# KORandi/bullet-js

Measured on AMD Instinct MI355X. Metric: CRDT field-merges/s, higher is better.
Workload: dtype int64

## Files before the change

bullet-js_amd/csrc/merge_kernels.h:

```cpp
#pragma once
#include "slot.h"
#include "../../include/bmx.h"

namespace bmx {

__device__ unsigned long long g_wait_ticks = 6000000000ull;
__device__ __forceinline__ bool wait_gave_up(unsigned long long t0, const uint32_t* status) {
  return wall_clock64() - t0 > g_wait_ticks || (__hip_atomic_load(status, __ATOMIC_RELAXED, __HIP_MEMORY_SCOPE_AGENT) & ST_SPIN) != 0;
}
constexpr int PART_MAX_SHARDS = 16;
struct SeqPtrs { unsigned long long* p[PART_MAX_SHARDS]; };

struct MergeArgs {
  Slot* slots;
  uint64_t nslots;
  const uint64_t* id;
  const uint32_t* field;
  const int64_t* ts;
  const int64_t* val;
  const bmx_delta_rec* recs;
  uint32_t n;
  uint32_t epoch;
  uint32_t* next;
  uint32_t* blk_follow;
  uint8_t* wflag;
  uint8_t* flags;
  uint32_t* slot_of;
  uint32_t* blk_info;
  unsigned long long* shard_ctr;
  uint32_t* status;
  uint32_t* blk_next;
  uint32_t blk_ents;
  uint32_t force;
  unsigned long long* started = nullptr;
  unsigned long long started_val = 0;
  const unsigned long long* k3_done = nullptr;
  unsigned long long k3_wait = 0;
  uint32_t* fld_out = nullptr;
  uint32_t log_slots = 0;
  SeqPtrs notify{}; uint32_t n_notify = 0; unsigned long long notify_value = 0;
  const unsigned long long* tail_words = nullptr; uint32_t tail_n = 0; unsigned long long tail_at_least = 0; unsigned long long* tail_diag = nullptr;
};

constexpr uint8_t W_NONE = 0, W_WINNER = 1, W_PENDING = 2, W_FIRST = 4;
constexpr uint8_t W_CREATED = 8;
constexpr uint8_t W_FIRSTWRITE = 16;
constexpr uint32_t BLK_COUNT = 0x7FFFFFFFu;
constexpr uint32_t CTR_SHARDS = 256, CTR_STRIDE = 16;

template <bool AOS>
__device__ __forceinline__ void load_delta(const MergeArgs& A, uint32_t j, uint64_t& id, uint32_t& field, int64_t& ts, int64_t& val) {
  if (AOS) {
    const uint4* p = reinterpret_cast<const uint4*>(A.recs + j);
    uint4 lo = p[0], hi = p[1];
    id = u64_of(lo.x, lo.y);
    field = lo.z;
    ts = i64_of(hi.x, hi.y);
    val = i64_of(hi.z, hi.w);
  } else {
    id = A.id[j]; field = A.field[j]; ts = A.ts[j]; val = A.val[j];
  }
}
template <bool AOS>
__device__ __forceinline__ void load_delta_tv(const MergeArgs& A, uint32_t j, int64_t& ts, int64_t& val) {
  if (AOS) {
    uint4 hi = reinterpret_cast<const uint4*>(A.recs + j)[1];
    ts = i64_of(hi.x, hi.y);
    val = i64_of(hi.z, hi.w);
  } else {
    ts = A.ts[j]; val = A.val[j];
  }
}

__device__ __forceinline__ void store_tv(Slot* sl, int64_t ts, int64_t val) {
  reinterpret_cast<uint4*>(sl)[1] = uint4_of((uint64_t)ts, (uint64_t)val);
}

template <bool UNIQUE>
__device__ __forceinline__ bool probe_or_insert(const MergeArgs& A, uint32_t tag, uint64_t id, uint32_t field, uint64_t& slot_out,
                                                bool& is_new, bool& created, uint32_t& prev_head, int64_t& cts, int64_t& cval) {
  created = false;
  ProbeSeq<4> ps(id, field, A.nslots);
  uint64_t p = 0;
  for (uint32_t round = 0; round < 256; ++round) {
    Slot* wait_on = nullptr;
    uint64_t s = 0;
    int done = 0;
    for (; p < A.nslots; ++p) {
      s = ps.slot();
      Slot* sl = A.slots + s;
      const uint4* q = reinterpret_cast<const uint4*>(sl);
      uint4 lo = q[0], hi = q[1];
      uint64_t sid = (uint64_t)lo.x | ((uint64_t)lo.y << 32);
      uint32_t sf = lo.z;
      bool fresh = false;
      if (sid == EMPTY_ID) {
        unsigned long long old = atomicCAS(reinterpret_cast<unsigned long long*>(&sl->id), (unsigned long long)EMPTY_ID, (unsigned long long)id);
        if (old == EMPTY_ID) {
          __hip_atomic_store(reinterpret_cast<unsigned long long*>(&sl->field), (unsigned long long)field | ((unsigned long long)(UNIQUE ? 0u : tag) << 32),
                             __ATOMIC_RELAXED, __HIP_MEMORY_SCOPE_AGENT);
          prev_head = 0;
          created = true;
          slot_out = s; is_new = true; cts = TS_NEW; cval = 0;
          done = 1;
          break;
        }
        sid = old;
        sf = FIELD_PENDING;
        fresh = true;
      }
      if (sid == id) {
        if (sf == FIELD_PENDING) { wait_on = sl; break; }
        if (sf == field) {
          int64_t t = (int64_t)((uint64_t)hi.x | ((uint64_t)hi.y << 32));
          slot_out = s;
          is_new = fresh || t == TS_NEW || ts_mark(t) == (tag >> IDX_BITS);
          cts = is_new ? TS_NEW : ts_value(t);
          cval = (int64_t)((uint64_t)hi.z | ((uint64_t)hi.w << 32));
          done = 1;
          break;
        }
      }
      ps.next();
    }
    if (done) return true;
    if (!wait_on) { atomicOr(A.status, ST_FULL); return false; }
    __builtin_amdgcn_wave_barrier();
    uint32_t sf = FIELD_PENDING, spins = 0;
    do {
      sf = __hip_atomic_load(&wait_on->field, __ATOMIC_RELAXED, __HIP_MEMORY_SCOPE_AGENT);
      if (sf != FIELD_PENDING) break;
      __builtin_amdgcn_s_sleep(1);
    } while (++spins < (1u << 22));
    if (sf == FIELD_PENDING) { atomicOr(A.status, ST_SPIN); return false; }
    if (sf == field) {
      slot_out = s; is_new = true; cts = TS_NEW; cval = 0;
      return true;
    }
    ps.next(); ++p;
  }
  atomicOr(A.status, ST_SPIN);
  return false;
}

template <int MODE, bool UNIQUE, bool TEAM = false>
__device__ __forceinline__ void decide_and_claim(const MergeArgs& A, const uint32_t j, const uint64_t s, const bool is_new, const bool created, uint32_t prev,
                                                 const int64_t cts, const int64_t cval, const int64_t a, const int64_t v,
                                                 uint32_t& fl, uint32_t& wf, bool& conflict) {
  const uint32_t tag = (A.epoch << IDX_BITS) | j;
  const int c = (is_new || A.force) ? 1 : lexcmp(a, v, cts, cval);
  if (c < 0) {
    fl = BMX_FLAG_CURRENT | (a < cts ? BMX_FLAG_HISTORICAL : 0u);
    return;
  }
  Slot* sl = A.slots + s;
  if (!TEAM && !created && !UNIQUE) prev = atomicExch(&sl->head, tag);
  if ((prev >> IDX_BITS) != A.epoch) {
    if (!UNIQUE) wf = W_FIRST;
    if (A.log_slots) A.slot_of[j] = (uint32_t)s;
    if (is_new) {
      const int64_t t0 = (MODE == BMX_INSERT_REFERENCE) ? 2 : a;
      store_tv(sl, t0 | ((int64_t)A.epoch << TS_MARK_SHIFT), v);
      wf |= W_WINNER | W_CREATED | W_FIRSTWRITE; fl = BMX_FLAG_INCOMING;
    } else if (c > 0) {
      if (!TEAM) store_tv(sl, a, v);
      wf |= W_WINNER; fl = BMX_FLAG_INCOMING;
    }
  } else {
    A.next[prev & IDX_MASK] = tag;
    A.slot_of[prev & IDX_MASK] = (uint32_t)s;
    A.blk_follow[(prev & IDX_MASK) >> 8] = A.epoch;
    wf = W_PENDING; conflict = true;
    fl = c > 0 ? BMX_FLAG_INCOMING : 0u;
  }
}

__device__ __forceinline__ uint32_t team_claim(const MergeArgs& A, const uint32_t j, const uint32_t s, const uint32_t field, const int64_t a, const int64_t v,
                                               const bool want, const bool wr) {
  const uint32_t lane = lane_id(), role = lane & 3u;
  const unsigned long long mw = __ballot(want), mv = __ballot(wr);
  uint32_t prev = 0;
#pragma unroll
  for (uint32_t p = 0; p < 4; p++) {
    if (!((mw >> (16u * p)) & 0xFFFFull)) continue;
    const uint32_t src = 16u * p + (lane >> 2);
    const uint32_t ss = (uint32_t)__shfl((int)s, (int)src), sf = (uint32_t)__shfl((int)field, (int)src);
    const uint64_t sa = u64_of((uint32_t)__shfl((int)lo32((uint64_t)a), (int)src), (uint32_t)__shfl((int)hi32((uint64_t)a), (int)src));
    const uint64_t sv = u64_of((uint32_t)__shfl((int)lo32((uint64_t)v), (int)src), (uint32_t)__shfl((int)hi32((uint64_t)v), (int)src));
    const bool on = role == 0 ? ((mw >> src) & 1ull) != 0 : (role != 3u && ((mv >> src) & 1ull) != 0);
    const uint64_t opnd = role == 0 ? u64_of(sf, (A.epoch << IDX_BITS) | (j - lane + src)) : (role == 1 ? sa : sv);
    unsigned long long old = 0;
    if (on) old = __hip_atomic_exchange(reinterpret_cast<unsigned long long*>(A.slots + ss) + 1 + role, (unsigned long long)opnd, __ATOMIC_RELAXED, __HIP_MEMORY_SCOPE_AGENT);
    const uint32_t got = (uint32_t)__shfl((int)hi32(old), (int)(4u * (lane & 15u)));
    if ((lane >> 4) == p) prev = got;
  }
  return prev;
}

template <bool AOS, int MODE, bool UNIQUE, int NT, bool TEAM = false>
__device__ __forceinline__ void probe_apply_body(const MergeArgs& A) {
  static_assert(!(TEAM && UNIQUE), "a unique-key batch claims nothing");
  const uint32_t j = blockIdx.x * (uint32_t)NT + threadIdx.x;
  if (A.started && j == 0) __hip_atomic_store(A.started, A.started_val, __ATOMIC_RELAXED, __HIP_MEMORY_SCOPE_AGENT);
  if (A.n_notify && j < A.n_notify && A.notify.p[j]) __hip_atomic_store(A.notify.p[j], A.notify_value, __ATOMIC_RELAXED, __HIP_MEMORY_SCOPE_SYSTEM);
  for (uint32_t t = j; t < A.blk_ents; t += gridDim.x * (uint32_t)NT) A.blk_next[t] = 0u;
  const bool active = j < A.n;
  uint64_t id = EMPTY_ID; uint32_t field = 0; int64_t a = 0, v = 0;
  if (active) load_delta<AOS>(A, j, id, field, a, v);
  if (A.fld_out && active) A.fld_out[j] = field;
  const bool pad = AOS && id == EMPTY_ID;
  const bool valid = active && id != EMPTY_ID && field != FIELD_PENDING && a >= 0 && a <= TS_MAX && ((v >= -VAL_MAX && v <= VAL_MAX) || (A.force && v == VAL_DELETED));
  if (active && !valid && !pad) atomicOr(A.status, ST_RANGE);
  uint32_t fl = 0, wf = W_NONE;
  bool conflict = false, created = false;
  if (TEAM) {
    bool is_new = false, located = false; int64_t cts = 0, cval = 0; uint64_t s = 0; uint32_t prev = 0;
    if (valid) located = probe_or_insert<UNIQUE>(A, (A.epoch << IDX_BITS) | j, id, field, s, is_new, created, prev, cts, cval);
    const int c = !located ? -1 : ((is_new || A.force) ? 1 : lexcmp(a, v, cts, cval));
    const bool want = c >= 0 && !created;
    const uint32_t got = team_claim(A, j, (uint32_t)s, field, a, v, want, want && c > 0 && !is_new);
    if (want) prev = got;
    if (located) decide_and_claim<MODE, UNIQUE, true>(A, j, s, is_new, created, prev, cts, cval, a, v, fl, wf, conflict);
  } else if (valid) {
    bool is_new; int64_t cts, cval; uint64_t s; uint32_t prev = 0;
    if (probe_or_insert<UNIQUE>(A, (A.epoch << IDX_BITS) | j, id, field, s, is_new, created, prev, cts, cval))
      decide_and_claim<MODE, UNIQUE>(A, j, s, is_new, created, prev, cts, cval, a, v, fl, wf, conflict);
  }
  if (active) {
    A.wflag[j] = (uint8_t)wf;
    if (A.flags) A.flags[j] = (uint8_t)fl;
  }
  const uint32_t nc = (uint32_t)__popcll(__ballot(created)), nx = (uint32_t)__popcll(__ballot(conflict));
  const uint32_t nw = (uint32_t)__popcll(__ballot((wf & W_WINNER) != 0));
  if (lane_id() == 0) {
    if (nw) atomicAdd(&A.blk_info[j >> 8], nw);
    if (nc | nx) {
      unsigned long long* ctr = A.shard_ctr + (size_t)((j >> 6) & (CTR_SHARDS - 1)) * CTR_STRIDE;
      if (nc) atomicAdd(ctr + 0, (unsigned long long)nc);
      if (nx) atomicAdd(ctr + 1, (unsigned long long)nx);
    }
  }
}

template <bool AOS, int MODE, bool UNIQUE, int NT, bool TEAM = false>
__global__ __launch_bounds__(NT) void k_probe_apply(MergeArgs A) { probe_apply_body<AOS, MODE, UNIQUE, NT, TEAM>(A); }
template <bool AOS, int MODE, bool UNIQUE, int NT, bool TEAM = false>
__global__ __launch_bounds__(NT) __attribute__((amdgpu_waves_per_eu(1, 6))) void k_probe_apply_w6(MergeArgs A) { probe_apply_body<AOS, MODE, UNIQUE, NT, TEAM>(A); }
template <bool AOS, int MODE, bool UNIQUE, int NT, bool TEAM = false>
__global__ __launch_bounds__(NT) __attribute__((amdgpu_waves_per_eu(1, 5))) void k_probe_apply_w5(MergeArgs A) { probe_apply_body<AOS, MODE, UNIQUE, NT, TEAM>(A); }
template <bool AOS, int MODE, bool UNIQUE, int NT, bool TEAM = false>
__global__ __launch_bounds__(NT) __attribute__((amdgpu_waves_per_eu(1, 4))) void k_probe_apply_w4(MergeArgs A) { probe_apply_body<AOS, MODE, UNIQUE, NT, TEAM>(A); }
template <bool AOS, int MODE, bool UNIQUE, int NT, bool TEAM = false>
__global__ __launch_bounds__(NT) __attribute__((amdgpu_waves_per_eu(1, 3))) void k_probe_apply_w3(MergeArgs A) { probe_apply_body<AOS, MODE, UNIQUE, NT, TEAM>(A); }


struct Top2 {
  int64_t t1 = INT64_MIN, v1 = INT64_MIN, t2 = INT64_MIN, v2 = INT64_MIN;
  uint32_t o1 = ~0u, o2 = ~0u;
  __device__ __forceinline__ void add(uint32_t idx, int64_t t, int64_t v) {
    int c1 = o1 == ~0u ? 1 : lexcmp(t, v, t1, v1);
    if (c1 > 0 || (c1 == 0 && idx < o1)) {
      if (o1 != ~0u) { int c2 = o2 == ~0u ? 1 : lexcmp(t1, v1, t2, v2); if (c2 > 0 || (c2 == 0 && o1 < o2)) { t2 = t1; v2 = v1; o2 = o1; } }
      t1 = t; v1 = v; o1 = idx;
    } else {
      int c2 = o2 == ~0u ? 1 : lexcmp(t, v, t2, v2);
      if (c2 > 0 || (c2 == 0 && idx < o2)) { t2 = t; v2 = v; o2 = idx; }
    }
  }
  __device__ __forceinline__ bool best_except(uint32_t skip, int64_t& t, int64_t& v, uint32_t& o) const {
    const bool use2 = o1 == skip;
    o = use2 ? o2 : o1;
    if (o == ~0u) return false;
    t = use2 ? t2 : t1; v = use2 ? v2 : v1;
    return true;
  }
};

template <bool AOS, int MODE>
__device__ __forceinline__ void resolve_one(const MergeArgs& A, const uint32_t j) {
  if (j >= A.n) return;
  const uint8_t wf = A.wflag[j];
  if (!(wf & W_FIRST)) return;
  uint32_t nx = A.next[j];
  if ((nx >> IDX_BITS) != A.epoch) return;
  int64_t t, v; load_delta_tv<AOS>(A, j, t, v);
  Slot* sl = A.slots + A.slot_of[j];
  const uint4 hi = reinterpret_cast<const uint4*>(sl)[1];
  const int64_t tsw = i64_of(hi.x, hi.y);
  const bool is_new = tsw == TS_NEW || ts_mark(tsw) == A.epoch;
  const uint32_t base_owner = (wf & W_WINNER) ? j : ~0u;
  int64_t bt, bv;
  uint32_t owner, created_by = ~0u;
  if (!is_new) {
    bt = t; bv = v; owner = base_owner;
    uint32_t idx = j, steps = 0;
    for (;;) {
      if (idx != j) {
        const bool gt = t > bt || (t == bt && v > bv);
        const bool eq = t == bt && v == bv;
        if (gt) { bt = t; bv = v; owner = idx; }
        else if (eq && owner != ~0u && idx < owner) owner = idx;
      }
      if ((nx >> IDX_BITS) != A.epoch) break;
      idx = nx & IDX_MASK;
      nx = A.next[idx]; load_delta_tv<AOS>(A, idx, t, v);
      if (++steps > A.n) { atomicOr(A.status, ST_SPIN); return; }
    }
  } else {
    uint32_t j0 = j;
    int64_t v_j0 = v, t_j0 = t;
    Top2 top;
    {
      uint32_t idx = j, steps = 0;
      for (;;) {
        if (idx <= j0) { j0 = idx; t_j0 = t; v_j0 = v; }
        top.add(idx, t, v);
        if ((nx >> IDX_BITS) != A.epoch) break;
        idx = nx & IDX_MASK;
        nx = A.next[idx]; load_delta_tv<AOS>(A, idx, t, v);
        if (++steps > A.n) { atomicOr(A.status, ST_SPIN); return; }
      }
    }
    bt = (MODE == BMX_INSERT_REFERENCE) ? 2 : t_j0; bv = v_j0; owner = j0; created_by = j0;
    int64_t tm, vm; uint32_t om;
    if (top.best_except(j0, tm, vm, om) && lexcmp(tm, vm, bt, bv) > 0) { bt = tm; bv = vm; owner = om; }
  }
  store_tv(sl, is_new ? (bt | ((int64_t)A.epoch << TS_MARK_SHIFT)) : bt, bv);
  if (base_owner != owner) {
    if (base_owner != ~0u) { A.wflag[base_owner] = W_NONE; atomicSub(&A.blk_info[base_owner >> 8], 1u); }
    if (owner != ~0u) {
      A.wflag[owner] = is_new ? (uint8_t)(W_WINNER | W_CREATED | (owner == created_by ? W_FIRSTWRITE : 0)) : W_WINNER; atomicAdd(&A.blk_info[owner >> 8], 1u);
      A.slot_of[owner] = A.slot_of[j];
    }
  } else if (is_new && owner != ~0u) {
    A.wflag[owner] = (uint8_t)(W_FIRST | W_WINNER | W_CREATED | (owner == created_by ? W_FIRSTWRITE : 0));
  }
  if (owner != ~0u && A.flags) A.flags[owner] = (uint8_t)BMX_FLAG_INCOMING;
}

template <bool AOS, int MODE>
__global__ __launch_bounds__(256) void k_resolve_lists(MergeArgs A) {
  if (A.blk_follow[blockIdx.x] == A.epoch) resolve_one<AOS, MODE>(A, blockIdx.x * 256u + threadIdx.x);
  if (A.k3_done && blockIdx.x == 0 && threadIdx.x == 0) {
    const unsigned long long t0 = wall_clock64();
    while (__hip_atomic_load(A.k3_done, __ATOMIC_RELAXED, __HIP_MEMORY_SCOPE_AGENT) < A.k3_wait) {
      __builtin_amdgcn_s_sleep(8);
      if (wait_gave_up(t0, A.status)) { atomicOr(A.status, ST_SPIN); break; }
    }
  }
  if (A.tail_n && blockIdx.x == 0 && threadIdx.x < A.tail_n) {
    const unsigned long long t0 = wall_clock64();
    unsigned long long seen;
    while ((seen = __hip_atomic_load(A.tail_words + threadIdx.x, __ATOMIC_RELAXED, __HIP_MEMORY_SCOPE_SYSTEM)) < A.tail_at_least) {
      __builtin_amdgcn_s_sleep(8);
      if (wait_gave_up(t0, A.status)) {
        if (A.tail_diag && !A.tail_diag[0]) { A.tail_diag[0] = (unsigned long long)(uintptr_t)(A.tail_words + threadIdx.x); A.tail_diag[1] = A.tail_at_least; A.tail_diag[2] = seen; }
        atomicOr(A.status, ST_SPIN);
        break;
      }
    }
  }
}

constexpr uint32_t STRICT_NO_ROW = 0xFFFFFFFFu;

template <bool AOS>
__global__ __launch_bounds__(256) void k_probe_link_strict(MergeArgs A) {
  const uint32_t j = blockIdx.x * 256u + threadIdx.x;
  const bool active = j < A.n;
  uint64_t id = EMPTY_ID; uint32_t field = 0; int64_t a = 0, v = 0;
  if (active) load_delta<AOS>(A, j, id, field, a, v);
  const bool pad = AOS && id == EMPTY_ID;
  const bool valid = active && id != EMPTY_ID && field != FIELD_PENDING && a >= 0 && a <= TS_MAX && ((v >= -VAL_MAX && v <= VAL_MAX) || (A.force && v == VAL_DELETED));
  if (active && !valid && !pad) atomicOr(A.status, ST_RANGE);
  uint32_t slot = STRICT_NO_ROW;
  bool conflict = false, created = false;
  if (valid) {
    bool is_new; int64_t cts, cval; uint64_t s; uint32_t prev = 0;
    const uint32_t tag = (A.epoch << IDX_BITS) | j;
    if (probe_or_insert<false>(A, tag, id, field, s, is_new, created, prev, cts, cval)) {
      if (!created) prev = atomicExch(&(A.slots + s)->head, tag);
      if ((prev >> IDX_BITS) == A.epoch) { A.next[j] = (A.epoch << IDX_BITS) | (prev & IDX_MASK); conflict = true; }
      slot = (uint32_t)s;
    }
  }
  {
    unsigned long long mc = __ballot(created), mx = __ballot(conflict);
    if (lane_id() == 0 && (mc | mx)) {
      unsigned long long* ctr = A.shard_ctr + (size_t)((blockIdx.x * 4u + (threadIdx.x >> 6)) & (CTR_SHARDS - 1)) * CTR_STRIDE;
      if (mc) atomicAdd(ctr + 0, (unsigned long long)__popcll(mc));
      if (mx) atomicAdd(ctr + 1, (unsigned long long)__popcll(mx));
    }
  }
  if (active) {
    A.slot_of[j] = slot;
    A.wflag[j] = W_NONE;
    if (A.flags) A.flags[j] = 0;
  }
  if (threadIdx.x == 0) A.blk_info[blockIdx.x] = 0;
}

template <bool AOS, int MODE, bool APPLY>
__global__ __launch_bounds__(256) void k_resolve_strict(MergeArgs A) {
  const uint32_t j = blockIdx.x * 256u + threadIdx.x;
  if (j >= A.n) return;
  const uint32_t slot = A.slot_of[j];
  if (slot == STRICT_NO_ROW) return;
  Slot* sl = A.slots + slot;
  const uint4* q = reinterpret_cast<const uint4*>(sl);
  const uint4 lo = q[0], hi = q[1];
  const uint32_t head = lo.w & IDX_MASK;
  if (APPLY && head != j) return;
  int64_t aj, vj; load_delta_tv<AOS>(A, j, aj, vj);
  const int64_t tsw = i64_of(hi.x, hi.y);
  const int64_t rval = i64_of(hi.z, hi.w);
  const bool is_new = tsw == TS_NEW;
  uint32_t j0 = ~0u; int64_t t_j0 = 0, v_j0 = 0;
  Top2 top;
  {
    uint32_t idx = head, steps = 0;
    for (;;) {
      int64_t t, v; load_delta_tv<AOS>(A, idx, t, v);
      uint32_t nx = A.next[idx];
      if (idx < j0) { j0 = idx; t_j0 = t; v_j0 = v; }
      if (APPLY || idx < j) top.add(idx, t, v);
      if ((nx >> IDX_BITS) != A.epoch) break;
      idx = nx & IDX_MASK;
      if (++steps > A.n) { atomicOr(A.status, ST_SPIN); return; }
    }
  }
  int64_t bt, bv; uint32_t owner;
  if (is_new) {
    bt = (MODE == BMX_INSERT_REFERENCE) ? 2 : t_j0; bv = v_j0; owner = j0;
    int64_t tm, vm; uint32_t om;
    if (top.best_except(j0, tm, vm, om) && lexcmp(tm, vm, bt, bv) > 0) { bt = tm; bv = vm; owner = om; }
  } else {
    bt = ts_value(tsw); bv = rval; owner = ~0u;
    if (top.o1 != ~0u && lexcmp(top.t1, top.v1, bt, bv) > 0) { bt = top.t1; bv = top.v1; owner = top.o1; }
  }
  if (APPLY) {
    if (owner != ~0u) {
      store_tv(sl, is_new ? (bt | ((int64_t)A.epoch << TS_MARK_SHIFT)) : bt, bv);
      A.wflag[owner] = (uint8_t)(W_WINNER | (is_new ? W_CREATED | (owner == j0 ? W_FIRSTWRITE : 0) : 0));
      atomicAdd(&A.blk_info[owner >> 8], 1u);
    }
  } else if (A.flags) {
    uint32_t fl;
    if (is_new && j == j0) {
      fl = BMX_FLAG_INCOMING;
    } else {
      int c = lexcmp(aj, vj, bt, bv);
      fl = c > 0 ? BMX_FLAG_INCOMING : (c == 0 ? 0u : (BMX_FLAG_CURRENT | (aj < bt ? BMX_FLAG_HISTORICAL : 0u)));
    }
    A.flags[j] = (uint8_t)fl;
  }
}

constexpr uint64_t TEAR_K = 0x5DEECE66DA5A5A5Aull;
template <bool SPLIT, bool TEAM = false>
__global__ __launch_bounds__(256) void k_selfcheck_tear(uint4* slots, uint32_t nslots, uint32_t iters, unsigned long long* torn, unsigned long long* reads) {
  typedef unsigned int u32x4 __attribute__((ext_vector_type(4)));
  const uint32_t gid = blockIdx.x * 256u + threadIdx.x;
  const bool writer = ((TEAM ? blockIdx.x >> 3 : blockIdx.x) & 1u) == 0;
  const uint32_t role = threadIdx.x & 3u;
  uint64_t x = (uint64_t)((TEAM && writer) ? gid >> 2 : gid) * 0x9E3779B97F4A7C15ull + 1;
  unsigned long long bad = 0, n = 0, sink = 0;
  for (uint32_t i = 0; i < iters; i++) {
    x = x * 6364136223846793005ull + 1442695040888963407ull;
    const uint32_t s = (uint32_t)(x >> 40) % nslots;
    uint4* p = slots + 2 * (size_t)s + 1;
    if (writer) {
      const uint64_t a = x, b = ~x ^ TEAR_K;
      if (TEAM) {
        unsigned long long* w = reinterpret_cast<unsigned long long*>(p) - 1 + role;
        const unsigned long long opnd = role == 0 ? u64_of(77u, gid) : (role == 1 ? a : b);
        if (SPLIT) {
          if (role == 0) sink ^= __hip_atomic_exchange(w, opnd, __ATOMIC_RELAXED, __HIP_MEMORY_SCOPE_AGENT);
          asm volatile("" ::: "memory");
          if (role == 1) sink ^= __hip_atomic_exchange(w, opnd, __ATOMIC_RELAXED, __HIP_MEMORY_SCOPE_AGENT);
          asm volatile("" ::: "memory");
          if (role == 2) sink ^= __hip_atomic_exchange(w, opnd, __ATOMIC_RELAXED, __HIP_MEMORY_SCOPE_AGENT);
        } else if (role != 3u) {
          sink ^= __hip_atomic_exchange(w, opnd, __ATOMIC_RELAXED, __HIP_MEMORY_SCOPE_AGENT);
        }
      } else if (SPLIT) { reinterpret_cast<volatile uint64_t*>(p)[0] = a; reinterpret_cast<volatile uint64_t*>(p)[1] = b; }
      else *p = uint4_of(a, b);
    } else {
      u32x4 v;
      if (blockIdx.x & 2u) v = __builtin_nontemporal_load(reinterpret_cast<const u32x4*>(p));
      else { v = *reinterpret_cast<const u32x4*>(p); asm volatile("" ::: "memory"); }
      const uint64_t a = u64_of(v.x, v.y), b = u64_of(v.z, v.w);
      if (!(a == 0 && b == 0) && b != (~a ^ TEAR_K)) bad++;
      n++;
    }
  }
  if (bad) atomicAdd(torn, bad);
  if (n | (sink == 0x0123456789ABCDEFull)) atomicAdd(reads, n);
}

__global__ __launch_bounds__(64) void k_placement_probe(Slot* slots, uint64_t nslots, uint32_t n, uint32_t salt, uint32_t team) {
  const uint32_t j = blockIdx.x * 64u + threadIdx.x;
  if (j >= n) return;
  const uint64_t h = mix64(((uint64_t)salt << 32) | j);
  const uint64_t s = __umul64hi(h, nslots);
  Slot* sl = slots + s;
  const uint4* q = reinterpret_cast<const uint4*>(sl);
  const uint4 lo = q[0], hi = q[1];
  if (team) {
    MergeArgs A{}; A.slots = slots; A.epoch = 1;
    const bool wr = ((lo.x ^ hi.x) & 7u) != 5u;
    const uint32_t prev = team_claim(A, j, (uint32_t)s, lo.z, (int64_t)u64_of(j, lo.y), (int64_t)u64_of(hi.z, hi.w), true, wr);
    if (prev == 0x9E3779B9u) sl->head = j;
    return;
  }
  const uint32_t prev = atomicExch(&sl->head, j);
  if (((lo.x ^ hi.x ^ prev) & 7u) != 5u)
    reinterpret_cast<uint4*>(sl)[1] = make_uint4(j, lo.y, hi.z, prev);
}

__global__ __launch_bounds__(256) void k_sweep_heads(Slot* slots, uint64_t nslots) {
  for (uint64_t s = (uint64_t)blockIdx.x * 256u + threadIdx.x; s < nslots; s += (uint64_t)gridDim.x * 256u) {
    slots[s].head = 0;
    int64_t t = slots[s].ts;
    if (t != TS_NEW && ts_mark(t)) slots[s].ts = ts_value(t);
  }
}

__global__ __launch_bounds__(256) void k_init_slots(Slot* slots, uint64_t nslots) {
  const uint4 lo = make_uint4(0xFFFFFFFFu, 0xFFFFFFFFu, FIELD_PENDING, 0u);
  const uint4 hi = make_uint4(0u, 0x80000000u, 0u, 0u);
  for (uint64_t s = (uint64_t)blockIdx.x * 256u + threadIdx.x; s < nslots; s += (uint64_t)gridDim.x * 256u) {
    uint4* q = reinterpret_cast<uint4*>(slots + s);
    q[0] = lo; q[1] = hi;
  }
}

__global__ __launch_bounds__(256) void k_rehash(const Slot* old_slots, uint64_t old_n, Slot* slots, uint64_t nslots, uint32_t* status) {
  for (uint64_t i = (uint64_t)blockIdx.x * 256u + threadIdx.x; i < old_n; i += (uint64_t)gridDim.x * 256u) {
    const uint4* q = reinterpret_cast<const uint4*>(old_slots + i);
    uint4 lo = q[0];
    uint64_t id = u64_of(lo.x, lo.y);
    if (id == EMPTY_ID) continue;
    uint4 hi = q[1];
    int64_t t = i64_of(hi.x, hi.y);
    if (t != TS_NEW) t = ts_value(t);
    ProbeSeq<4> ps(id, lo.z, nslots);
    bool done = false;
    for (uint64_t p = 0; p < nslots && !done; ++p) {
      Slot* sl = slots + ps.slot();
      unsigned long long old = atomicCAS(reinterpret_cast<unsigned long long*>(&sl->id), (unsigned long long)EMPTY_ID, (unsigned long long)id);
      if (old == EMPTY_ID) {
        sl->field = lo.z; sl->head = 0;
        reinterpret_cast<uint4*>(sl)[1] = make_uint4(lo32((uint64_t)t), hi32((uint64_t)t), hi.z, hi.w);
        done = true;
      } else {
        ps.next();
      }
    }
    if (!done) atomicOr(status, ST_FULL);
  }
}

__global__ __launch_bounds__(256) void k_get_rows(const Slot* slots, uint64_t nslots, uint32_t n, const uint64_t* id,
                                                  const uint32_t* field, int64_t* ts, int64_t* val, uint8_t* found) {
  uint32_t j = blockIdx.x * 256u + threadIdx.x;
  if (j >= n) return;
  uint64_t kid = id[j]; uint32_t kf = field[j];
  ProbeSeq<4> ps(kid, kf, nslots);
  uint8_t f = 0; int64_t t = 0, v = 0;
  for (uint64_t p = 0; p < nslots; ++p) {
    const uint4* q = reinterpret_cast<const uint4*>(slots + ps.slot());
    uint4 lo = q[0];
    uint64_t sid = u64_of(lo.x, lo.y);
    if (sid == EMPTY_ID) break;
    if (sid == kid && lo.z == kf) {
      uint4 hi = q[1];
      t = i64_of(hi.x, hi.y);
      v = i64_of(hi.z, hi.w);
      f = t != TS_NEW;
      t = ts_value(t);
      break;
    }
    ps.next();
  }
  ts[j] = t; val[j] = v; found[j] = f;
}

__global__ void k_seq_signal(unsigned long long* seq, unsigned long long value) {
  if (threadIdx.x == 0) __hip_atomic_store(seq, value, __ATOMIC_RELEASE, __HIP_MEMORY_SCOPE_AGENT);
}
__global__ void k_seq_wait(const unsigned long long* seq, unsigned long long at_least, uint32_t* status, unsigned long long* diag) {
  if (threadIdx.x != 0) return;
  const unsigned long long t0 = wall_clock64();
  unsigned long long seen;
  while ((seen = __hip_atomic_load(seq, __ATOMIC_ACQUIRE, __HIP_MEMORY_SCOPE_AGENT)) < at_least) {
    __builtin_amdgcn_s_sleep(8);
    if (wait_gave_up(t0, status)) {
      if (diag && !diag[0]) { diag[0] = (unsigned long long)(uintptr_t)seq; diag[1] = at_least; diag[2] = seen; }
      atomicOr(status, ST_SPIN);
      return;
    }
  }
}

__global__ void k_seq_wait_all(const unsigned long long* words, uint32_t n, unsigned long long at_least, uint32_t* status, unsigned long long* diag) {
  const uint32_t k = threadIdx.x;
  if (k >= n) return;
  const unsigned long long t0 = wall_clock64();
  unsigned long long seen;
  while ((seen = __hip_atomic_load(words + k, __ATOMIC_RELAXED, __HIP_MEMORY_SCOPE_SYSTEM)) < at_least) {
    __builtin_amdgcn_s_sleep(8);
    if (wait_gave_up(t0, status)) {
      if (diag && !diag[0]) { diag[0] = (unsigned long long)(uintptr_t)(words + k); diag[1] = at_least; diag[2] = seen; }
      atomicOr(status, ST_SPIN);
      return;
    }
  }
}
__global__ void k_seq_signal_multi(SeqPtrs w, uint32_t n, unsigned long long value) {
  if (threadIdx.x < n && w.p[threadIdx.x]) __hip_atomic_store(w.p[threadIdx.x], value, __ATOMIC_RELAXED, __HIP_MEMORY_SCOPE_SYSTEM);
}


constexpr int PART_BLOCKS = 1024;
constexpr uint32_t PART_TILE = 1024;
struct PartOut {
  bmx_delta_rec* base[PART_MAX_SHARDS];
  uint32_t split;
  uint32_t aux_base;
  const unsigned long long* wait_words = nullptr; uint32_t n_wait = 0; unsigned long long wait_at_least = 0; unsigned long long* wait_diag = nullptr;
};

__device__ __forceinline__ uint32_t owner_of_dev(uint64_t id, uint32_t nshards) { return (uint32_t)__umul64hi(owner_hash(id), (uint64_t)nshards); }

__global__ __launch_bounds__(256) void k_part_count(const uint64_t* id, uint32_t n, uint32_t nshards, uint32_t per_block,
                                                    uint32_t* counts , uint8_t* owner_out ) {
  __shared__ uint32_t wtot[4][PART_MAX_SHARDS];
  const uint32_t lane = threadIdx.x & 63, w = threadIdx.x >> 6;
  uint32_t lo = blockIdx.x * per_block, hi = min(n, lo + per_block);
  uint32_t mine = 0;
  for (uint32_t t0 = lo; t0 < hi; t0 += 256) {
    uint32_t j = t0 + threadIdx.x;
    uint32_t g = j < hi ? owner_of_dev(id[j], nshards) : 0xFFFFFFFFu;
    if (j < hi) owner_out[j] = (uint8_t)g;
    for (uint32_t gg = 0; gg < nshards; gg++) {
      uint32_t c = (uint32_t)__popcll(__ballot(g == gg));
      if (lane == gg) mine += c;
    }
  }
  if (lane < PART_MAX_SHARDS) wtot[w][lane] = mine;
  __syncthreads();
  if (threadIdx.x < nshards) counts[threadIdx.x * PART_BLOCKS + blockIdx.x] = wtot[0][threadIdx.x] + wtot[1][threadIdx.x] + wtot[2][threadIdx.x] + wtot[3][threadIdx.x];
}

__global__ __launch_bounds__(256) void k_part_scatter(const uint64_t* id, const uint32_t* field, const int64_t* ts, const int64_t* val,
                                                      const uint8_t* owner, uint32_t n, uint32_t nshards, uint32_t per_block, const uint32_t* counts,
                                                      bmx_delta_rec* out, unsigned long long* totals, uint32_t slab, uint32_t* status, PartOut po) {
  __shared__ uint32_t base[PART_MAX_SHARDS];
  __shared__ uint32_t tot[PART_MAX_SHARDS];
  __shared__ uint32_t red[PART_MAX_SHARDS][2];
  __shared__ uint4 stage[PART_TILE * 2];
  __shared__ __attribute__((aligned(16))) uint32_t F[PART_MAX_SHARDS * 16 + 4];
  const uint32_t lane = threadIdx.x & 63, w = threadIdx.x >> 6;
  const uint32_t lo = blockIdx.x * per_block, hi = min(n, lo + per_block);
  uint64_t kid[4], rt[4], rv[4]; uint32_t rf[4], g[4];
  auto load_tile = [&](uint32_t t0) {
#pragma unroll
    for (int i = 0; i < 4; i++) {
      const uint32_t j = t0 + (uint32_t)i * 256u + threadIdx.x;
      const bool act = j < hi;
      kid[i] = act ? id[j] : EMPTY_ID; rf[i] = act ? field[j] : 0u; rt[i] = act ? (uint64_t)ts[j] : 0ull; rv[i] = act ? (uint64_t)val[j] : 0ull;
      g[i] = act ? (uint32_t)owner[j] : 0xFFu;
    }
  };
  if (lo < hi) load_tile(lo);
  if (po.n_wait) {
    __shared__ uint32_t gave_up;
    if (threadIdx.x == 0) gave_up = 0;
    __syncthreads();
    if (threadIdx.x < po.n_wait) {
      const unsigned long long t0 = wall_clock64();
      unsigned long long seen;
      while ((seen = __hip_atomic_load(po.wait_words + threadIdx.x, __ATOMIC_RELAXED, __HIP_MEMORY_SCOPE_SYSTEM)) < po.wait_at_least) {
        __builtin_amdgcn_s_sleep(8);
        if (wait_gave_up(t0, status)) {
          if (po.wait_diag && !po.wait_diag[0]) { po.wait_diag[0] = (unsigned long long)(uintptr_t)(po.wait_words + threadIdx.x); po.wait_diag[1] = po.wait_at_least; po.wait_diag[2] = seen; }
          atomicOr(status, ST_SPIN); gave_up = 1u;
          break;
        }
      }
    }
    __syncthreads();
    if (gave_up) return;
  }
  for (uint32_t gs = w; gs < nshards; gs += 4) {
    const uint4* cg = reinterpret_cast<const uint4*>(counts + gs * PART_BLOCKS);
    uint32_t before = 0, all = 0;
#pragma unroll
    for (uint32_t k = 0; k < PART_BLOCKS / 256; k++) {
      const uint32_t b4 = k * 64 + lane;
      const uint4 c = cg[b4];
      const uint32_t b0 = b4 * 4;
      all += c.x + c.y + c.z + c.w;
      before += (b0 < blockIdx.x ? c.x : 0u) + (b0 + 1 < blockIdx.x ? c.y : 0u) + (b0 + 2 < blockIdx.x ? c.z : 0u) + (b0 + 3 < blockIdx.x ? c.w : 0u);
    }
    before = wave_incl_scan_u32(before); all = wave_incl_scan_u32(all);
    if (lane == 63) { red[gs][0] = before; red[gs][1] = all; }
  }
  __syncthreads();
  if (threadIdx.x < nshards) {
    tot[threadIdx.x] = red[threadIdx.x][1];
    if (blockIdx.x == 0) {
      totals[threadIdx.x] = red[threadIdx.x][1];
      if (slab && red[threadIdx.x][1] > slab) atomicOr(status, ST_SLAB);
    }
  }
  __syncthreads();
  if (threadIdx.x < nshards) {
    uint32_t gg = threadIdx.x, start = 0;
    if (slab) start = gg * slab;
    else for (uint32_t x = 0; x < gg; x++) start += tot[x];
    base[gg] = start + red[gg][0];
  }
  const uint32_t nwords = (nshards + 3) >> 2;
  for (uint32_t t0 = lo; t0 < hi; t0 += PART_TILE) {
    if (t0 != lo) load_tile(t0);
    uint32_t rk[4];
#pragma unroll
    for (int i = 0; i < 4; i++) {
      rk[i] = 0;
      const uint32_t c = (uint32_t)i * 4u + w;
      for (uint32_t k = 0; k < nwords; k++) {
        const uint32_t sh = (g[i] & 3u) * 8u;
        const bool mine = (g[i] >> 2) == k;
        const uint32_t incl = wave_incl_scan_u32(mine ? (1u << sh) : 0u);
        if (mine) rk[i] = ((incl >> sh) & 0xFFu) - 1u;
        const uint32_t totw = (uint32_t)__builtin_amdgcn_readlane((int)incl, 63);
        if (lane < 4 && 4 * k + lane < nshards) F[(4 * k + lane) * 16 + c] = (totw >> (8u * lane)) & 0xFFu;
      }
    }
    __syncthreads();
    if (w == 0) {
      const bool live = lane * 4 < nshards * 16;
      uint4 x = live ? reinterpret_cast<const uint4*>(F)[lane] : make_uint4(0u, 0u, 0u, 0u);
      const uint32_t sum = x.x + x.y + x.z + x.w;
      const uint32_t incl = wave_incl_scan_u32(sum);
      const uint32_t e = incl - sum;
      reinterpret_cast<uint4*>(F)[lane] = make_uint4(e, e + x.x, e + x.x + x.y, e + x.x + x.y + x.z);
      if (lane == 63) F[PART_MAX_SHARDS * 16] = incl;
    }
    __syncthreads();
    uint32_t grow = 0;
    if (threadIdx.x < nshards) grow = F[(threadIdx.x + 1) * 16] - F[threadIdx.x * 16];
#pragma unroll
    for (int i = 0; i < 4; i++) {
      if (g[i] != 0xFFu) {
        const uint32_t p = F[g[i] * 16 + (uint32_t)i * 4u + w] + rk[i];
        stage[2 * p] = make_uint4(lo32(kid[i]), hi32(kid[i]), rf[i], po.aux_base + t0 + (uint32_t)i * 256u + threadIdx.x);
        stage[2 * p + 1] = uint4_of((uint64_t)rt[i], (uint64_t)rv[i]);
      }
    }
    __syncthreads();
    for (uint32_t gg = 0; gg < nshards; gg++) {
      const uint32_t s0 = F[gg * 16], e0 = F[(gg + 1) * 16], b = base[gg];
      uint4* out16 = po.split ? reinterpret_cast<uint4*>(po.base[gg]) - 2 * (size_t)gg * slab : reinterpret_cast<uint4*>(out);
      for (uint32_t q = 2 * s0 + threadIdx.x; q < 2 * e0; q += 256) {
        const uint32_t pos = b + ((q >> 1) - s0);
        if (!slab || pos - gg * slab < slab)
          out16[2 * (size_t)pos + (q & 1)] = stage[q];
      }
    }
    __syncthreads();
    if (threadIdx.x < nshards) base[threadIdx.x] += grow;
  }
  if (slab) {
    const uint4 padlo = make_uint4(0xFFFFFFFFu, 0xFFFFFFFFu, FIELD_PENDING, 0u), padhi = make_uint4(0u, 0u, 0u, 0u);
    for (uint32_t g = 0; g < nshards; g++) {
      uint32_t used = min(tot[g], slab);
      for (uint32_t p = used + blockIdx.x * 256u + threadIdx.x; p < slab; p += PART_BLOCKS * 256u) {
        uint4* q = reinterpret_cast<uint4*>((po.split ? po.base[g] : out + (size_t)g * slab) + p);
        q[0] = padlo; q[1] = padhi;
      }
    }
  }
}

}
```

Measured before the change: 11.58 billion.

## Probe hash table a whole 4-slot line per trip instead of one slot

Rewrites probe_or_insert to load an entire 128-byte line of four slots at once and pick the first empty, pending or matching slot with bitmask logic (line_walk), rather than issuing one load round-trip per probed slot. This is meant to cut dependent memory latency on probe chains. The strict kernel is pinned to the old per-slot version, and a standalone microbenchmark compares the two. The line walk reads a snapshot of all four slots, so it has to handle CAS races by retrying within the line.

```diff
diff --git a/bench_micro/line_probe_micro.hip b/bench_micro/line_probe_micro.hip
--- /dev/null
+++ b/bench_micro/line_probe_micro.hip
@@ -0,0 +1,151 @@
+#include <hip/hip_runtime.h>
+#include <cstdio>
+#include <cstdlib>
+#include <cstdint>
+#include <vector>
+#include <algorithm>
+#include "../bullet-js_amd/csrc/slot.h"
+#include "../bullet-js_amd/csrc/line_walk.h"
+using namespace bmx;
+#define CK(x) do{hipError_t e=(x); if(e!=hipSuccess){printf("HIP error %s at %d\n",hipGetErrorString(e),__LINE__); exit(1);} }while(0)
+
+constexpr uint32_t ABSENT = 0x80000000u;
+__host__ __device__ inline uint64_t key_id(uint64_t i) { return mix64(i + 0x1234567ull) >> 1; }
+__host__ __device__ inline uint32_t key_field(uint64_t i) { return (uint32_t)(mix64(i * 3 + 1) & 7u) * 0x61C88647u + 12345u; }
+
+__global__ __launch_bounds__(256) void k_fill_rows(Slot* slots, uint64_t nslots, uint64_t nrows, unsigned long long* failed) {
+  const uint64_t i = (uint64_t)blockIdx.x * 256u + threadIdx.x;
+  if (i >= nrows) return;
+  const uint64_t id = key_id(i); const uint32_t field = key_field(i);
+  ProbeSeq<4> ps(id, field, nslots);
+  for (uint64_t p = 0; p < nslots; ++p, ps.next()) {
+    Slot* sl = slots + ps.slot();
+    if (atomicCAS(reinterpret_cast<unsigned long long*>(&sl->id), (unsigned long long)EMPTY_ID, (unsigned long long)id) == EMPTY_ID) {
+      sl->field = field; sl->head = 0; sl->ts = (int64_t)(i & 1023); sl->val = (int64_t)i;
+      return;
+    }
+  }
+  atomicAdd(failed, 1ull);
+}
+__global__ void k_clear(uint4* t, size_t n16) {
+  size_t i = (size_t)blockIdx.x * blockDim.x + threadIdx.x; const size_t st = (size_t)gridDim.x * blockDim.x;
+  for (; i < n16; i += st) t[i] = (i & 1) ? make_uint4(0u, 0x80000000u, 0u, 0u) : make_uint4(~0u, ~0u, 0u, 0u);
+}
+__global__ __launch_bounds__(256) void k_gen(uint64_t* id, uint32_t* field, int64_t* ts, int64_t* val, uint32_t n, uint64_t nrows, uint64_t seed) {
+  const uint32_t j = blockIdx.x * 256u + threadIdx.x;
+  if (j >= n) return;
+  const uint64_t r = mix64(j + seed * 0x9E3779B97F4A7C15ull);
+  const bool absent = (r % 10) == 0;
+  const uint64_t i = absent ? (1ull << 40) + (r >> 8) : __umul64hi(mix64(r), nrows);
+  id[j] = key_id(i); field[j] = key_field(i); ts[j] = (int64_t)(r & 1023); val[j] = (int64_t)(r >> 40);
+}
+
+template <int V>
+__global__ __launch_bounds__(64) void k_lookup(const Slot* slots, uint64_t nslots, const uint64_t* cid, const uint32_t* cfield, const int64_t* cts, const int64_t* cval,
+                                               uint32_t n, uint32_t* out, uint8_t* sink) {
+  const uint32_t j = blockIdx.x * 64u + threadIdx.x;
+  if (j >= n) return;
+  const uint64_t id = cid[j]; const uint32_t field = cfield[j]; const int64_t a = cts[j], v = cval[j];
+  ProbeSeq<4> ps(id, field, nslots);
+  uint32_t res = ~0u; uint4 hi = make_uint4(0, 0, 0, 0);
+  if (V == 0) {
+    for (uint64_t p = 0; p < nslots; ++p) {
+      const uint64_t s = ps.slot();
+      const uint4* q = reinterpret_cast<const uint4*>(slots + s);
+      const uint4 lo = q[0], h = q[1];
+      const uint64_t sid = (uint64_t)lo.x | ((uint64_t)lo.y << 32);
+      if (sid == EMPTY_ID) { res = (uint32_t)s | ABSENT; break; }
+      if (sid == id && lo.z == field) { res = (uint32_t)s; hi = h; break; }
+      ps.next();
+    }
+  } else {
+    uint64_t line = ps.line;
+    for (uint64_t p = 0; p < nslots; p += 4) {
+      const uint4* q = reinterpret_cast<const uint4*>(slots + line * 4);
+      const uint4 l0 = q[0], h0 = q[1], l1 = q[2], h1 = q[3], l2 = q[4], h2 = q[5], l3 = q[6], h3 = q[7];
+      const LineWalk w = line_walk((uint64_t)l0.x | ((uint64_t)l0.y << 32), l0.z, (uint64_t)l1.x | ((uint64_t)l1.y << 32), l1.z,
+                                   (uint64_t)l2.x | ((uint64_t)l2.y << 32), l2.z, (uint64_t)l3.x | ((uint64_t)l3.y << 32), l3.z, id, field, ps.c);
+      if (w.verdict != LW_NEXT_LINE) {
+        const uint32_t i = (ps.c + w.k) & 3u;
+        res = (uint32_t)(line * 4 + i);
+        if (w.verdict == LW_EMPTY) res |= ABSENT;
+        else hi = make_uint4(lw_pick(i, h0.x, h1.x, h2.x, h3.x), lw_pick(i, h0.y, h1.y, h2.y, h3.y), lw_pick(i, h0.z, h1.z, h2.z, h3.z), lw_pick(i, h0.w, h1.w, h2.w, h3.w));
+        break;
+      }
+      line = (line + 1 == ps.nlines) ? 0 : line + 1;
+    }
+  }
+  out[j] = res;
+  sink[j] = (uint8_t)(hi.x ^ hi.y ^ hi.z ^ hi.w ^ (uint32_t)a ^ (uint32_t)v);
+}
+
+struct Batch { uint64_t* id; uint32_t* field; int64_t* ts; int64_t* val; };
+static void launch(int v, const Slot* slots, uint64_t nslots, const Batch& b, uint32_t n, uint32_t* out, uint8_t* sink) {
+  const dim3 g((n + 63) / 64), blk(64);
+  if (v == 0) hipLaunchKernelGGL((k_lookup<0>), g, blk, 0, 0, slots, nslots, b.id, b.field, b.ts, b.val, n, out, sink);
+  else hipLaunchKernelGGL((k_lookup<1>), g, blk, 0, 0, slots, nslots, b.id, b.field, b.ts, b.val, n, out, sink);
+}
+
+int main() {
+  const uint32_t n = 1u << 20;
+  const uint64_t nslots = 44ull << 20;
+  const size_t bytes = nslots * 32;
+  const int NB = 10;
+  Slot* slots; CK(hipMalloc(&slots, bytes));
+  Batch b[NB];
+  for (int k = 0; k < NB; k++) { CK(hipMalloc(&b[k].id, (size_t)n * 8)); CK(hipMalloc(&b[k].field, (size_t)n * 4)); CK(hipMalloc(&b[k].ts, (size_t)n * 8)); CK(hipMalloc(&b[k].val, (size_t)n * 8)); }
+  uint32_t* out; uint8_t* sink; unsigned long long* failed;
+  CK(hipMalloc(&out, (size_t)n * 4)); CK(hipMalloc(&sink, n)); CK(hipMalloc(&failed, 8));
+  hipEvent_t e0, e1; CK(hipEventCreate(&e0)); CK(hipEventCreate(&e1));
+  const char* names[2] = {"A one slot per trip", "B whole line, one trip"};
+  std::vector<uint32_t> h(n);
+  int rc = 0;
+  uint64_t rows_in = 0;
+  for (int li = 0; li < 2; li++) {
+    const uint64_t nrows = (li == 0 ? 11ull : 22ull) << 20;
+    CK(hipMemset(failed, 0, 8));
+    hipLaunchKernelGGL(k_clear, dim3(4096), dim3(256), 0, 0, reinterpret_cast<uint4*>(slots), bytes / 16);
+    hipLaunchKernelGGL(k_fill_rows, dim3((unsigned)((nrows + 255) / 256)), dim3(256), 0, 0, slots, nslots, nrows, failed);
+    CK(hipDeviceSynchronize());
+    rows_in = nrows;
+    unsigned long long hf = 0; CK(hipMemcpy(&hf, failed, 8, hipMemcpyDeviceToHost));
+    if (hf) { printf("fill failed for %llu rows\n", hf); return 1; }
+    for (int k = 0; k < NB; k++) hipLaunchKernelGGL(k_gen, dim3(n / 256), dim3(256), 0, 0, b[k].id, b[k].field, b[k].ts, b[k].val, n, nrows, (uint64_t)(li * 100 + k + 1));
+    CK(hipDeviceSynchronize());
+    unsigned long long sum[2] = {0, 0}; uint32_t nabs[2] = {0, 0}, nmiss[2] = {0, 0};
+    for (int v = 0; v < 2; v++) {
+      CK(hipMemset(out, 0xEE, (size_t)n * 4));
+      launch(v, slots, nslots, b[0], n, out, sink); CK(hipDeviceSynchronize());
+      CK(hipMemcpy(h.data(), out, (size_t)n * 4, hipMemcpyDeviceToHost));
+      for (uint32_t j = 0; j < n; j++) { sum[v] += (unsigned long long)h[j] * (j | 1u); nabs[v] += (h[j] & ABSENT) != 0 && h[j] != ~0u; nmiss[v] += h[j] == ~0u; }
+    }
+    const double load = (double)rows_in / (double)nslots;
+    printf("load %.2f (%llu rows in %llu slots) | checksum A %016llx B %016llx %s | absent A %u B %u | table exhausted A %u B %u\n", load, (unsigned long long)rows_in,
+           (unsigned long long)nslots, sum[0], sum[1], sum[0] == sum[1] ? "agree" : "DIFFER", nabs[0], nabs[1], nmiss[0], nmiss[1]);
+    if (sum[0] != sum[1] || nmiss[0] || nmiss[1]) rc = 1;
+    for (int v = 0; v < 2; v++) for (int k = 0; k < 3; k++) launch(v, slots, nslots, b[k], n, out, sink);
+    CK(hipDeviceSynchronize());
+    const int REPEATS = 7;
+    std::vector<float> t[2];
+    for (int rep = 0; rep < REPEATS; rep++) for (int v = 0; v < 2; v++) {
+      CK(hipEventRecord(e0));
+      for (int k = 0; k < NB; k++) launch(v, slots, nslots, b[k], n, out, sink);
+      CK(hipEventRecord(e1)); CK(hipEventSynchronize(e1));
+      float ms; CK(hipEventElapsedTime(&ms, e0, e1)); t[v].push_back(ms / NB * 1000.f);
+    }
+    float mn[2], mx[2];
+    for (int v = 0; v < 2; v++) {
+      mn[v] = *std::min_element(t[v].begin(), t[v].end()); mx[v] = *std::max_element(t[v].begin(), t[v].end());
+      printf("load %.2f | %-22s | us per 1M, %d repeats of %d launches:", load, names[v], REPEATS, NB);
+      for (float x : t[v]) printf(" %.1f", x);
+      printf(" | min %.1f max %.1f range %.1f\n", mn[v], mx[v], mx[v] - mn[v]);
+    }
+    if (li == 0) {
+      const bool pass = mx[1] < mn[0];
+      printf("gate (load 0.25: every B repeat faster than every A repeat): %s (slowest B %.1f, fastest A %.1f)\n", pass ? "PASS" : "FAIL", mx[1], mn[0]);
+      if (!pass && !rc) rc = 2;
+    }
+    fflush(stdout);
+  }
+  return rc;
+}
diff --git a/bullet-js_amd/csrc/line_walk.h b/bullet-js_amd/csrc/line_walk.h
--- /dev/null
+++ b/bullet-js_amd/csrc/line_walk.h
@@ -0,0 +1,54 @@
+#pragma once
+#include <stdint.h>
+
+#ifndef __HIPCC__
+#ifndef __host__
+#define __host__
+#endif
+#ifndef __device__
+#define __device__
+#endif
+#endif
+
+namespace bmx {
+
+constexpr uint64_t LW_EMPTY_ID = ~0ull;
+constexpr uint32_t LW_FIELD_PENDING = 0xFFFFFFFFu;
+
+constexpr uint32_t LW_EMPTY = 0;
+constexpr uint32_t LW_FOUND = 1;
+constexpr uint32_t LW_WAIT = 2;
+constexpr uint32_t LW_PASS = 3;
+constexpr uint32_t LW_NEXT_LINE = 4;
+
+struct LineWalk {
+  uint32_t k;
+  uint32_t verdict;
+};
+
+__host__ __device__ inline uint32_t lw_slot_verdict(uint64_t sid, uint32_t sf, uint64_t id, uint32_t field) {
+  return sid == LW_EMPTY_ID ? LW_EMPTY : (sid != id ? LW_PASS : (sf == LW_FIELD_PENDING ? LW_WAIT : (sf == field ? LW_FOUND : LW_PASS)));
+}
+
+__host__ __device__ inline uint32_t lw_pick(uint32_t i, uint32_t a0, uint32_t a1, uint32_t a2, uint32_t a3) {
+  return (a0 & (0u - (uint32_t)(i == 0))) | (a1 & (0u - (uint32_t)(i == 1))) | (a2 & (0u - (uint32_t)(i == 2))) | (a3 & (0u - (uint32_t)(i == 3)));
+}
+
+__host__ __device__ inline LineWalk line_walk(uint64_t id0, uint32_t f0, uint64_t id1, uint32_t f1, uint64_t id2, uint32_t f2, uint64_t id3, uint32_t f3,
+                                              uint64_t id, uint32_t field, uint32_t c, uint32_t from = 0) {
+  const uint32_t empty = (uint32_t)(id0 == LW_EMPTY_ID) | ((uint32_t)(id1 == LW_EMPTY_ID) << 1) | ((uint32_t)(id2 == LW_EMPTY_ID) << 2) | ((uint32_t)(id3 == LW_EMPTY_ID) << 3);
+  const uint32_t own = ((uint32_t)(id0 == id) | ((uint32_t)(id1 == id) << 1) | ((uint32_t)(id2 == id) << 2) | ((uint32_t)(id3 == id) << 3)) & ~empty;
+  const uint32_t pend = own & ((uint32_t)(f0 == LW_FIELD_PENDING) | ((uint32_t)(f1 == LW_FIELD_PENDING) << 1) | ((uint32_t)(f2 == LW_FIELD_PENDING) << 2) | ((uint32_t)(f3 == LW_FIELD_PENDING) << 3));
+  const uint32_t match = own & ~pend & ((uint32_t)(f0 == field) | ((uint32_t)(f1 == field) << 1) | ((uint32_t)(f2 == field) << 2) | ((uint32_t)(f3 == field) << 3));
+  const uint32_t sh = c & 3u, ahead = (0xFu << (from > 4u ? 4u : from)) & 0xFu;
+  const uint32_t e = ((empty | (empty << 4)) >> sh) & ahead, w = ((pend | (pend << 4)) >> sh) & ahead, m = ((match | (match << 4)) >> sh) & ahead;
+  const uint32_t decide = e | w | m;
+  const uint32_t lowest = decide & (0u - decide);
+  const uint32_t k = (lowest >> 1) - (lowest >> 3);
+  LineWalk r;
+  r.k = decide ? k : 4u;
+  r.verdict = !decide ? LW_NEXT_LINE : ((e & lowest) ? LW_EMPTY : ((w & lowest) ? LW_WAIT : LW_FOUND));
+  return r;
+}
+
+}
diff --git a/bullet-js_amd/csrc/merge_kernels.h b/bullet-js_amd/csrc/merge_kernels.h
--- a/bullet-js_amd/csrc/merge_kernels.h
+++ b/bullet-js_amd/csrc/merge_kernels.h
@@ -1,5 +1,6 @@
 #pragma once
 #include "slot.h"
+#include "line_walk.h"
 #include "../../include/bmx.h"
 
 namespace bmx {
@@ -79,6 +80,84 @@
 template <bool UNIQUE>
 __device__ __forceinline__ bool probe_or_insert(const MergeArgs& A, uint32_t tag, uint64_t id, uint32_t field, uint64_t& slot_out,
                                                 bool& is_new, bool& created, uint32_t& prev_head, int64_t& cts, int64_t& cval) {
+  static_assert(LW_EMPTY_ID == EMPTY_ID && LW_FIELD_PENDING == FIELD_PENDING, "line_walk.h and slot.h name the same reserved values");
+  created = false;
+  const ProbeSeq<4> ps(id, field, A.nslots);
+  const uint32_t nslots = (uint32_t)A.nslots, nlines = (uint32_t)ps.nlines;
+  uint32_t line = (uint32_t)ps.line;
+  uint32_t k = 0;
+  uint32_t p = 0;
+  for (uint32_t round = 0; round < 256; ++round) {
+    Slot* wait_on = nullptr;
+    uint32_t s = 0;
+    int done = 0;
+    while (p < nslots) {
+      const uint4* q = reinterpret_cast<const uint4*>(A.slots + (uint64_t)line * 4);
+      const uint4 l0 = q[0], h0 = q[1], l1 = q[2], h1 = q[3], l2 = q[4], h2 = q[5], l3 = q[6], h3 = q[7];
+      const uint64_t i0 = (uint64_t)l0.x | ((uint64_t)l0.y << 32), i1 = (uint64_t)l1.x | ((uint64_t)l1.y << 32);
+      const uint64_t i2 = (uint64_t)l2.x | ((uint64_t)l2.y << 32), i3 = (uint64_t)l3.x | ((uint64_t)l3.y << 32);
+      for (;;) {
+        const LineWalk w = line_walk(i0, l0.z, i1, l1.z, i2, l2.z, i3, l3.z, id, field, ps.c, k);
+        p += w.k - k;
+        k = w.k;
+        if (w.verdict == LW_NEXT_LINE) break;
+        const uint32_t i = (ps.c + k) & 3u;
+        s = line * 4 + i;
+        Slot* sl = A.slots + s;
+        if (w.verdict == LW_EMPTY) {
+          unsigned long long old = atomicCAS(reinterpret_cast<unsigned long long*>(&sl->id), (unsigned long long)EMPTY_ID, (unsigned long long)id);
+          if (old == EMPTY_ID) {
+            __hip_atomic_store(reinterpret_cast<unsigned long long*>(&sl->field), (unsigned long long)field | ((unsigned long long)(UNIQUE ? 0u : tag) << 32),
+                               __ATOMIC_RELAXED, __HIP_MEMORY_SCOPE_AGENT);
+            prev_head = 0;
+            created = true;
+            slot_out = s; is_new = true; cts = TS_NEW; cval = 0;
+            done = 1;
+            break;
+          }
+          if (old == id) { wait_on = sl; break; }
+          ++k; ++p;
+          continue;
+        }
+        if (w.verdict == LW_WAIT) { wait_on = sl; break; }
+        const uint32_t tx = lw_pick(i, h0.x, h1.x, h2.x, h3.x), ty = lw_pick(i, h0.y, h1.y, h2.y, h3.y);
+        const uint32_t vx = lw_pick(i, h0.z, h1.z, h2.z, h3.z), vy = lw_pick(i, h0.w, h1.w, h2.w, h3.w);
+        int64_t t = (int64_t)((uint64_t)tx | ((uint64_t)ty << 32));
+        slot_out = s;
+        is_new = t == TS_NEW || ts_mark(t) == (tag >> IDX_BITS);
+        cts = is_new ? TS_NEW : ts_value(t);
+        cval = (int64_t)((uint64_t)vx | ((uint64_t)vy << 32));
+        done = 1;
+        break;
+      }
+      if (done || wait_on) break;
+      line = (line + 1 == nlines) ? 0 : line + 1;
+      k = 0;
+    }
+    if (done) return true;
+    if (!wait_on) { atomicOr(A.status, ST_FULL); return false; }
+    __builtin_amdgcn_wave_barrier();
+    uint32_t sf = FIELD_PENDING, spins = 0;
+    do {
+      sf = __hip_atomic_load(&wait_on->field, __ATOMIC_RELAXED, __HIP_MEMORY_SCOPE_AGENT);
+      if (sf != FIELD_PENDING) break;
+      __builtin_amdgcn_s_sleep(1);
+    } while (++spins < (1u << 22));
+    if (sf == FIELD_PENDING) { atomicOr(A.status, ST_SPIN); return false; }
+    if (sf == field) {
+      slot_out = s; is_new = true; cts = TS_NEW; cval = 0;
+      return true;
+    }
+    ++k; ++p;
+    if (k == 4) { line = (line + 1 == nlines) ? 0 : line + 1; k = 0; }
+  }
+  atomicOr(A.status, ST_SPIN);
+  return false;
+}
+
+template <bool UNIQUE>
+__device__ __forceinline__ bool probe_or_insert_by_slot(const MergeArgs& A, uint32_t tag, uint64_t id, uint32_t field, uint64_t& slot_out,
+                                                bool& is_new, bool& created, uint32_t& prev_head, int64_t& cts, int64_t& cval) {
   created = false;
   ProbeSeq<4> ps(id, field, A.nslots);
   uint64_t p = 0;
@@ -378,7 +457,7 @@
   if (valid) {
     bool is_new; int64_t cts, cval; uint64_t s; uint32_t prev = 0;
     const uint32_t tag = (A.epoch << IDX_BITS) | j;
-    if (probe_or_insert<false>(A, tag, id, field, s, is_new, created, prev, cts, cval)) {
+    if (probe_or_insert_by_slot<false>(A, tag, id, field, s, is_new, created, prev, cts, cval)) {
       if (!created) prev = atomicExch(&(A.slots + s)->head, tag);
       if ((prev >> IDX_BITS) == A.epoch) { A.next[j] = (A.epoch << IDX_BITS) | (prev & IDX_MASK); conflict = true; }
       slot = (uint32_t)s;
```

Result: slower. 6.856 billion (-40.8%).
